# vccheng2001/DeepVCP-Pointcloud-Registration

Hardware: AMD Instinct MI355X
Metric: pairs/sec (full DeepVCP forward) at N=16384, K=64; rot/trans error vs ref (higher is better)
Workload: dtype f32

## Files before the change

### deepvcp-pointcloud-registration_amd/csrc/knn_tiled.hip

```cpp
#include "common.h"
#include "morton.h"

namespace dvcp {

constexpr int kTile = 16;
constexpr int kMaxTiles = 1024;
constexpr uint32_t kTileIdBits = 0x3FFu;
constexpr int kTiledThreads = 256;
constexpr int kBoxBatch = 1;

struct TiledLayout {
  float4* sorted;
  float4* tbox;
  float4* qsorted;
  uint32_t* qbins;
  uint32_t* qbox;
};

inline int64_t align256(int64_t x) { return (x + 255) & ~int64_t(255); }

inline TiledLayout tiled_layout(void* ws, int B, int M, int Q) {
  const int64_t T = ceil_div(M, kTile);
  char* p = static_cast<char*>(ws);
  TiledLayout L;
// ... 386 lines not shown
          const float dx = c[4 * j] - qx, dy = c[4 * j + 1] - qy, dz = c[4 * j + 2] - qz;
          d2v[j] = (dx * dx + dy * dy) + dz * dz;
          piv[j] = __float_as_uint(c[4 * j + 3]);
          const uint64_t pk = (static_cast<uint64_t>(__float_as_uint(d2v[j])) << 32) | piv[j];
          const bool cand = act & (d2v[j] < __builtin_huge_valf()) & (pk < kkey);
          todo |= __ballot(cand) != 0 ? (1u << j) : 0u;
        }
        while (todo) {
          const int j = __builtin_ctz(todo);
          todo &= todo - 1;
          const float d2 = d2v[j];
          const uint32_t pi = piv[j];
          const uint64_t pk = (static_cast<uint64_t>(__float_as_uint(d2)) << 32) | pi;
          const bool cand = act & (d2 < __builtin_huge_valf()) & (pk < kkey);
          const uint64_t m = __ballot(cand);
          if (m == 0) continue;
          ins |= m;
          const uint64_t pkc = cand ? pk : ~0ull;
          bool lt[KT];
#pragma unroll
          for (int u = 0; u < KT; ++u) lt[u] = pkc < DVCP_KK(u);
#pragma unroll
          for (int u = KT - 1; u > 0; --u) {
            kh[u] = lt[u - 1] ? kh[u - 1] : (lt[u] ? __float_as_uint(d2) : kh[u]);
            kl[u] = lt[u - 1] ? kl[u - 1] : (lt[u] ? pi : kl[u]);
          }
          kh[0] = lt[0] ? __float_as_uint(d2) : kh[0];
          kl[0] = lt[0] ? pi : kl[0];
          kkey = live ? (KT == 1 ? DVCP_KK(0) : DVCP_KK(kq)) : 0ull;
          kth = __uint_as_float(static_cast<uint32_t>(kkey >> 32));
        }
      }
      if (ins != 0) wkth = wave_max_nonneg(kth);
      }
    }
  }
  if (!live) return;
  const int64_t o = (static_cast<int64_t>(b) * Q + q) * k;
#pragma unroll
  for (int t = 0; t < KT; ++t) {
    if (t < k) {
      const bool ok = DVCP_KK(t) != kEmpty;
      const float d2 = __uint_as_float(kh[t]);
      const int i = static_cast<int>(kl[t]);
      if (dist) dist[o + t] = ok ? sqrt_rn(d2) : __builtin_huge_valf();
      if (idx) idx[o + t] = ok ? i : -1;
      if (idx64) idx64[o + t] = ok ? i : -1;
    }
  }
#undef DVCP_KK
}


#ifndef DVCP_KNN_SORD
#define DVCP_KNN_SORD 1
#endif
#ifndef DVCP_KNN_STAGE_OUT
#define DVCP_KNN_STAGE_OUT 2
#endif
constexpr int kSelBufN = 16;
constexpr int kSelSortN = 16;
constexpr int kSordWords = (kMaxTiles + 2) / 3;
#ifndef DVCP_KNN_CHUNK
#define DVCP_KNN_CHUNK 1
#endif
#ifndef DVCP_KNN_SLOAD
#define DVCP_KNN_SLOAD 1
#endif

constexpr double kKeyEmpty = __builtin_bit_cast(double, 0x3FF0000000000000ull | (0x7F800000ull << 14) | 0x3FFFull);
__device__ __forceinline__ double key_pack(float d2, uint32_t index) {
  return __builtin_bit_cast(double, 0x3FF0000000000000ull | (static_cast<uint64_t>(__float_as_uint(d2)) << 14) |
                                        static_cast<uint64_t>(index & 0x3FFFu));
}
__device__ __forceinline__ float key_d2(double kd) {
  return __uint_as_float(static_cast<uint32_t>((__builtin_bit_cast(uint64_t, kd) >> 14) & 0x7FFFFFFFull));
}
__device__ __forceinline__ int key_index(double kd) {
  return static_cast<int>(__builtin_bit_cast(uint64_t, kd) & 0x3FFFull);
}
__device__ __forceinline__ void key_ce_f64(double& a, double& b, bool asc) {
  const double lo = __builtin_fmin(a, b), hi = __builtin_fmax(a, b);
  a = asc ? lo : hi;
  b = asc ? hi : lo;
}

__device__ __forceinline__ void key_ce(uint32_t& ah, uint32_t& al, uint32_t& bh, uint32_t& bl, bool asc) {
  const uint64_t a = (static_cast<uint64_t>(ah) << 32) | al, b = (static_cast<uint64_t>(bh) << 32) | bl;
  const bool sw = asc ? (b < a) : (a < b);
  const uint32_t th = ah, tl = al;
  ah = sw ? bh : ah;
  al = sw ? bl : al;
  bh = sw ? th : bh;
  bl = sw ? tl : bl;
}

template <int R>
__global__ __launch_bounds__(kTiledThreads) __attribute__((amdgpu_waves_per_eu(3))) void knn_sel_query_kernel(const float4* __restrict__ sorted,
                                                                      const float4* __restrict__ tbox,
                                                                      const float4* __restrict__ qsorted, int M,
                                                                      int Q, int k,
                                                                      float* __restrict__ dist,
                                                                      int32_t* __restrict__ idx,
                                                                      int64_t* __restrict__ idx64, int B8) {
  constexpr int KT = 32;
  const int lane = threadIdx.x & 63, wave = threadIdx.x >> 6;
  int b = blockIdx.y, bx = blockIdx.x;
  if ((B8 & 1) != 0) {
    const int lin = static_cast<int>(blockIdx.y * gridDim.x + blockIdx.x);
    const int xo = lin & 7, slot = lin >> 3;
    b = xo + 8 * (slot / static_cast<int>(gridDim.x));
    bx = slot % static_cast<int>(gridDim.x);
  }
  const int T = (M + kTile - 1) / kTile;
  __shared__ uint3 hbox[kMaxTiles];
  __shared__ uint32_t sord[kTiledThreads / kWave][kSordWords];
  __shared__ double sbuf[kTiledThreads / kWave][kSelBufN][kWave];
  __shared__ float4 stile[kTiledThreads / kWave][kTile];
  {
    const float4* tbg = tbox + static_cast<int64_t>(b) * T * 2;
    for (int i = threadIdx.x; i < T; i += kTiledThreads) hbox[i] = pack_hbox(tbg[2 * i], tbg[2 * i + 1]);
    __syncthreads();
  }
  const int sq0 = __builtin_amdgcn_readfirstlane((bx * (kTiledThreads / kWave) + wave) * kWave);
  const int sq = sq0 + lane;
  if (sq0 >= Q) return;
  const bool live = sq < Q;
  const float4 qrow = live ? qsorted[static_cast<int64_t>(b) * Q + sq] : make_float4(0.f, 0.f, 0.f, 0.f);
  const float qx = qrow.x, qy = qrow.y, qz = qrow.z;
  auto out_row = [&]() {
    const int sqn = sq0 + knn_fresh_lane();
    return __float_as_int(qsorted[static_cast<int64_t>(b) * Q + sqn].w);
  };
  float wl[3] = {live ? qx : __builtin_huge_valf(), live ? qy : __builtin_huge_valf(),
                 live ? qz : __builtin_huge_valf()};
  float wh[3] = {live ? qx : -__builtin_huge_valf(), live ? qy : -__builtin_huge_valf(),
                 live ? qz : -__builtin_huge_valf()};
#pragma unroll
  for (int a = 0; a < 3; ++a) {
    wl[a] = __int_as_float(__builtin_amdgcn_readfirstlane(__float_as_int(-wave_max_nonneg_signed(-wl[a]))));
    wh[a] = __int_as_float(__builtin_amdgcn_readfirstlane(__float_as_int(wave_max_nonneg_signed(wh[a]))));
  }
  uint32_t keys[R];
#pragma unroll
  for (int r = 0; r < R; ++r) {
    const int t = r * 64 + lane;
    if (t < T) {
      const float lb = hbox_lb2(hbox[t], wl[0], wl[1], wl[2], wh[0], wh[1], wh[2]);
      keys[r] = (__float_as_uint(lb) & ~kTileIdBits) | static_cast<uint32_t>(t);
    } else {
      keys[r] = 0xFFFFFFFFu;
    }
  }
  wave_bitonic<R>(keys);

  double tk[KT];
#pragma unroll
  for (int t = 0; t < KT; ++t) tk[t] = kKeyEmpty;
  float kth = live ? __builtin_huge_valf() : 0.0f;
  float wkth = wave_max_nonneg(kth);
  int fill = 0;
  double(*mybuf)[kWave] = sbuf[wave];
#ifdef DVCP_KNN_DIAG
  uint64_t dg_t0 = __builtin_readcyclecounter(), dg_merge_clk = 0, dg_skip_clk = 0, dg_prev = 0;
  int dg_kind = -1;
  int dg_scanned = 0, dg_active = 0, dg_merges = 0, dg_appends = 0;
#endif

  auto merge = [&]() {
    const int n = static_cast<int>(wave_umax_i(static_cast<uint32_t>(fill)));
    if (n == 0) return;
#ifdef DVCP_KNN_DIAG
    const uint64_t dg_m0 = __builtin_readcyclecounter();
    ++dg_merges;
#endif
    double bk[kSelSortN];
#pragma unroll
    for (int i = 0; i < kSelSortN; ++i) {
      bk[i] = kKeyEmpty;
      if (i < kSelBufN && i < n) {
        const double e = mybuf[i][lane];
        bk[i] = i < fill ? e : bk[i];
      }
    }
#pragma unroll
    for (int kk = 2; kk <= kSelSortN; kk <<= 1)
#pragma unroll
      for (int j = kk >> 1; j > 0; j >>= 1)
#pragma unroll
        for (int i = 0; i < kSelSortN; ++i) {
          const int l = i ^ j;
          if (l > i) key_ce_f64(bk[i], bk[l], (i & kk) == 0);
        }
#pragma unroll
    for (int i = KT - kSelSortN; i < KT; ++i) tk[i] = __builtin_fmin(tk[i], bk[KT - 1 - i]);
#pragma unroll
    for (int j = KT >> 1; j > 0; j >>= 1)
#pragma unroll
      for (int i = 0; i < KT; ++i) {
        const int l = i ^ j;
        if (l > i) key_ce_f64(tk[i], tk[l], true);
      }
    kth = live ? key_d2(tk[KT - 1]) : 0.0f;
    wkth = wave_max_nonneg(kth);
    fill = 0;
#ifdef DVCP_KNN_DIAG
    dg_merge_clk += __builtin_readcyclecounter() - dg_m0;
// ... 29 lines not shown
#pragma unroll
    for (int j = 0; j < kTile; ++j) {
      c[3 * j] = bc(4 * j);
      c[3 * j + 1] = bc(4 * j + 1);
      c[3 * j + 2] = bc(4 * j + 2);
    }
#endif
    auto d2_of = [&](int j) {
      const float dx = c[3 * j] - qx, dy = c[3 * j + 1] - qy, dz = c[3 * j + 2] - qz;
      return (dx * dx + dy * dy) + dz * dz;
    };
    uint32_t cm = 0;
    const float kf = fminf(kth, __builtin_bit_cast(float, 0x7F7FFFFFu));
#pragma unroll
    for (int j = 0; j < kTile; ++j) cm |= (act && d2_of(j) <= kf) ? (1u << j) : 0u;
    if (wave_umax_i(static_cast<uint32_t>(fill + __popc(cm))) > static_cast<uint32_t>(kSelBufN)) {
      merge();
      const float kf2 = fminf(kth, __builtin_bit_cast(float, 0x7F7FFFFFu));
#pragma unroll
      for (int j = 0; j < kTile; ++j) cm &= d2_of(j) <= kf2 ? ~0u : ~(1u << j);
    }
    if (__ballot(cm != 0) != 0) {
#if DVCP_KNN_SLOAD
      reinterpret_cast<float*>(stile[wave])[lane] = P[static_cast<int64_t>(t) * (4 * kTile) + lane];
#else
      reinterpret_cast<float*>(stile[wave])[lane] = v_cur;
#endif
      __builtin_amdgcn_wave_barrier();
      uint32_t my = cm;
      while (__ballot(my != 0) != 0) {
        if (my != 0) {
          const int j = __builtin_ctz(my);
          my &= my - 1;
#ifdef DVCP_KNN_DIAG
          ++dg_appends;
#endif
          const float4 pt = stile[wave][j];
          const float dx = pt.x - qx, dy = pt.y - qy, dz = pt.z - qz;
          mybuf[fill][lane] = key_pack((dx * dx + dy * dy) + dz * dz, __float_as_uint(pt.w));
          ++fill;
        }
      }
      __builtin_amdgcn_wave_barrier();
    }
  };
  auto visit = [&](uint32_t key) {
    const int t = static_cast<int>(key & kTileIdBits);
    const float lbq = hbox_lb2(hbox[t], qx, qy, qz, qx, qy, qz);
    float v = 0.0f;
    if (__ballot(live & (lbq <= kth)) != 0) v = P[static_cast<int64_t>(t) * (4 * kTile) + lane];
    visit_loaded(key, lbq, v);
  };

#if DVCP_KNN_CHUNK
  constexpr int kKnnSub = 4, kSubLanes = kWave / kKnnSub;
  float gl[3] = {wl[0], wl[1], wl[2]}, gh[3] = {wh[0], wh[1], wh[2]};
  {
    float a[3] = {live ? qx : __builtin_huge_valf(), live ? qy : __builtin_huge_valf(),
                  live ? qz : __builtin_huge_valf()};
    float z[3] = {live ? qx : -__builtin_huge_valf(), live ? qy : -__builtin_huge_valf(),
                  live ? qz : -__builtin_huge_valf()};
#pragma unroll
    for (int ax = 0; ax < 3; ++ax)
#pragma unroll
      for (int off = kSubLanes / 2; off > 0; off >>= 1) {
        a[ax] = fminf(a[ax], __shfl_xor(a[ax], off, kWave));
        z[ax] = fmaxf(z[ax], __shfl_xor(z[ax], off, kWave));
      }
#pragma unroll
    for (int ax = 0; ax < 3; ++ax) {
      gl[ax] = a[ax];
      gh[ax] = z[ax];
    }
  }
  __shared__ float4 sgbox[kTiledThreads / kWave][kKnnSub][2];
  if ((lane & (kSubLanes - 1)) == 0) {
    sgbox[wave][lane / kSubLanes][0] = make_float4(gl[0], gl[1], gl[2], 0.0f);
    sgbox[wave][lane / kSubLanes][1] = make_float4(gh[0], gh[1], gh[2], 0.0f);
  }
#if DVCP_KNN_SORD
  for (int i = lane; i < kSordWords; i += kWave) sord[wave][i] = 0u;
  __builtin_amdgcn_wave_barrier();
#pragma unroll
  for (int r = 0; r < R; ++r) {
    const int p = r * 64 + lane;
    if (p < T) atomicOr(&sord[wave][p / 3], (keys[r] & kTileIdBits) << (10 * (p % 3)));
  }
  __builtin_amdgcn_wave_barrier();
#endif
  bool stop = false;
#pragma unroll 1
  for (int base = 0; base < T && !stop; base += kWave) {
    const bool inr = base + lane < T;
#if DVCP_KNN_SORD
    const int pos = base + lane;
    const int tt = inr ? static_cast<int>((sord[wave][pos / 3] >> (10 * (pos % 3))) & kTileIdBits) : 0;
    const uint3 hb = hbox[tt];
    const uint32_t mykey = inr ? (__float_as_uint(hbox_lb2(hb, wl[0], wl[1], wl[2], wh[0], wh[1], wh[2])) &
                                  ~kTileIdBits) | static_cast<uint32_t>(tt)
                               : 0xFFFFFFFFu;
#else
    const uint32_t mykey = keys[base >> 6];
    const int tt = inr ? static_cast<int>(mykey & kTileIdBits) : 0;
    const uint3 hb = hbox[tt < T ? tt : 0];
#endif
    const float klb = __uint_as_float(mykey & ~kTileIdBits);
    const uint64_t over = __ballot(!inr || klb > wkth);
    const int lim = over ? __builtin_ctzll(over) : kWave;
    float gk = kth;
#pragma unroll
    for (int off = kSubLanes / 2; off > 0; off >>= 1) gk = fmaxf(gk, __shfl_xor(gk, off, kWave));
    float gks[kKnnSub];
#pragma unroll
    for (int g = 0; g < kKnnSub; ++g) gks[g] = __int_as_float(__builtin_amdgcn_readlane(__float_as_int(gk), g * kSubLanes));
    const float blx = half_lo(hb.x), bly = half_hi(hb.x), blz = half_lo(hb.y);
    const float bhx = half_hi(hb.y), bhy = half_lo(hb.z), bhz = half_hi(hb.z);
    bool pass = false;
#pragma unroll
    for (int g = 0; g < kKnnSub; ++g) {
      const float4 lo = sgbox[wave][g][0], hi = sgbox[wave][g][1];
      pass |= box_box_lb2(lo.x, lo.y, lo.z, hi.x, hi.y, hi.z, blx, bly, blz, bhx, bhy, bhz) <= gks[g];
    }
    uint64_t cand = __ballot(pass && inr) & (lim >= kWave ? ~0ull : ((1ull << lim) - 1ull));
    if (lim < kWave) stop = true;
    while (cand) {
      const int i = __builtin_ctzll(cand);
      cand &= cand - 1ull;
      const uint32_t key = static_cast<uint32_t>(__builtin_amdgcn_readlane(static_cast<int>(mykey), i));
      if (__uint_as_float(key & ~kTileIdBits) > wkth) {
        stop = true;
        break;
      }
      visit(key);
    }
  }
#else
  uint32_t key_next = T > 0 ? static_cast<uint32_t>(__builtin_amdgcn_readlane(static_cast<int>(keys[0]), 0)) : 0u;
#pragma unroll 1
  for (int pos = 0; pos < T; ++pos) {
#ifdef DVCP_KNN_DIAG
    {
      const uint64_t now = __builtin_readcyclecounter();
      if (dg_kind == 0) dg_skip_clk += now - dg_prev;
      dg_prev = now;
      dg_kind = 0;
    }
#endif
    const uint32_t key = key_next;
    if (pos + 1 < T)
      key_next = static_cast<uint32_t>(__builtin_amdgcn_readlane(static_cast<int>(keys[(pos + 1) >> 6]), (pos + 1) & 63));
    if (__uint_as_float(key & ~kTileIdBits) > wkth) break;
    visit(key);
  }
#endif
  merge();
#ifdef DVCP_KNN_DIAG
  const uint64_t dg_total = __builtin_readcyclecounter() - dg_t0;
  uint32_t app_sum = static_cast<uint32_t>(dg_appends);
  for (int off = 32; off > 0; off >>= 1) app_sum += __shfl_xor(app_sum, off, kWave);
#endif
#ifndef DVCP_KNN_DIAG
  if constexpr (DVCP_KNN_STAGE_OUT == 2) {
    if (dist && idx && !idx64 && k == KT) {
      if (!live) return;
      const int qo = out_row();
      float4* dr = reinterpret_cast<float4*>(dist + (static_cast<int64_t>(b) * Q + qo) * 32);
      int4* ir = reinterpret_cast<int4*>(idx + (static_cast<int64_t>(b) * Q + qo) * 32);
#pragma unroll
      for (int v = 0; v < KT / 4; ++v) {
        float dv[4];
        int iv[4];
#pragma unroll
        for (int e = 0; e < 4; ++e) {
          const double kv = tk[4 * v + e];
          const bool ok = kv != kKeyEmpty;
          dv[e] = ok ? sqrt_rn(key_d2(kv)) : __builtin_huge_valf();
          iv[e] = ok ? key_index(kv) : -1;
        }
        dr[v] = make_float4(dv[0], dv[1], dv[2], dv[3]);
        ir[v] = make_int4(iv[0], iv[1], iv[2], iv[3]);
      }
      return;
    }
  }
  if constexpr (DVCP_KNN_STAGE_OUT == 1) {
    if (dist && idx && !idx64 && k == KT) {
      const int qo = live ? out_row() : -1;
      float* stage = reinterpret_cast<float*>(sbuf[wave]);
#pragma unroll
      for (int part = 0; part < 2; ++part) {
#pragma unroll
        for (int half = 0; half < 2; ++half) {
          if ((lane >> 5) == half) {
#pragma unroll
            for (int t = 0; t < KT; ++t) {
              const bool ok = tk[t] != kKeyEmpty;
              const float v = part == 0 ? (ok ? sqrt_rn(key_d2(tk[t])) : __builtin_huge_valf())
                                        : __int_as_float(ok ? key_index(tk[t]) : -1);
              stage[(lane & 31) * 33 + t] = v;
            }
          }
          __builtin_amdgcn_wave_barrier();
          __builtin_amdgcn_fence(__ATOMIC_ACQ_REL, "wavefront");
#pragma unroll
          for (int it = 0; it < 4; ++it) {
            const int row = it * 8 + (lane >> 3), piece = lane & 7;
            const int rq = __shfl(qo, half * 32 + row, kWave);
            const float* sr = stage + row * 33 + 4 * piece;
            const float4 v = make_float4(sr[0], sr[1], sr[2], sr[3]);
            if (rq >= 0) {
              float* dst = part == 0 ? dist : reinterpret_cast<float*>(idx);
              reinterpret_cast<float4*>(dst + (static_cast<int64_t>(b) * Q + rq) * 32)[piece] = v;
            }
          }
          __builtin_amdgcn_wave_barrier();
          __builtin_amdgcn_fence(__ATOMIC_ACQ_REL, "wavefront");
        }
      }
      return;
    }
  }
#endif
  if (!live) return;
  const int qo = out_row();
  const int64_t o = (static_cast<int64_t>(b) * Q + qo) * k;
#ifdef DVCP_KNN_DIAG
  if (lane == 0 && dist && k == 32) {
    dist[o + 0] = static_cast<float>(dg_scanned);
    dist[o + 1] = static_cast<float>(dg_active);
    dist[o + 2] = static_cast<float>(dg_merges);
    dist[o + 3] = static_cast<float>(app_sum);
    dist[o + 4] = static_cast<float>(dg_total);
    dist[o + 5] = static_cast<float>(dg_merge_clk);
    dist[o + 6] = static_cast<float>(dg_skip_clk);
    dist[o + 31] = -12345.0f;
    return;
  }
#endif
#pragma unroll
  for (int t = 0; t < KT; ++t) {
    if (t < k) {
      const bool ok = tk[t] != kKeyEmpty;
      const float d2 = key_d2(tk[t]);
      const int i = key_index(tk[t]);
      if (dist) dist[o + t] = ok ? sqrt_rn(d2) : __builtin_huge_valf();
      if (idx) idx[o + t] = ok ? i : -1;
      if (idx64) idx64[o + t] = ok ? i : -1;
    }
  }
}

}

extern "C" int64_t dvcp_knn_tiled_workspace_bytes(int B, int M, int Q) {
  if (B < 0 || M < 0 || Q < 0) return -1;
  const int64_t T = dvcp::ceil_div(M, dvcp::kTile);
  return dvcp::align256(16 * int64_t(B) * T * dvcp::kTile) + dvcp::align256(32 * int64_t(B) * T) +
         dvcp::align256(16 * int64_t(B) * Q) + dvcp::align256(dvcp::tiled_zeroed_bytes(B));
}

static int knn_tiled_impl(int dtype, const void* ref, int64_t rb, int64_t rc, int64_t rn, int M, const void* qry,
                          int64_t qb, int64_t qc, int64_t qn, int Q, int B, int k, void* workspace, float* dist,
                          int32_t* idx, int64_t* idx64, void* stream, bool insertion) {
  DVCP_REQUIRE(ref && qry && workspace, "dvcp_knn_tiled: null pointer");
  DVCP_REQUIRE(k > 0 && k <= 32 && M >= 0 && Q >= 0 && B >= 0 && B <= 65535, "dvcp_knn_tiled: bad sizes");
  DVCP_REQUIRE(M <= dvcp::kMaxTiles * dvcp::kTile, "dvcp_knn_tiled: M=%d > %d", M, dvcp::kMaxTiles * dvcp::kTile);
  DVCP_REQUIRE(dtype == DVCP_F32 || dtype == DVCP_F64, "dvcp_knn_tiled: bad dtype %d", dtype);
  if (B == 0 || Q == 0) return DVCP_OK;
  hipStream_t st = static_cast<hipStream_t>(stream);
  const dvcp::TiledLayout L = dvcp::tiled_layout(workspace, B, M, Q);
  if (hipMemsetAsync(L.qbins, 0, dvcp::tiled_zeroed_bytes(B), st) != hipSuccess) {
    dvcp::set_error("dvcp_knn_tiled: memset failed");
    return DVCP_EHIP;
  }
  const dim3 qgrid(dvcp::ceil_div(Q, dvcp::kQSortItems), B), bgrid(1 + qgrid.x, B);
  if (dtype == DVCP_F32) {
    const dvcp::PointsView<float> qv{static_cast<const float*>(qry), qb, qc, qn};
    hipLaunchKernelGGL((dvcp::knn_qbox_kernel<float>), qgrid, dim3(dvcp::kBuildThreads), 0, st, qv, Q, L.qbox);
    hipLaunchKernelGGL((dvcp::knn_qhist_kernel<float>), qgrid, dim3(dvcp::kBuildThreads), 0, st, qv, Q, L.qbox,
                       L.qbins);
    hipLaunchKernelGGL(dvcp::knn_qscan_kernel, dim3(B), dim3(dvcp::kBuildThreads), 0, st, L.qbins);
    hipLaunchKernelGGL((dvcp::knn_tiled_build_kernel<float>), bgrid, dim3(dvcp::kBuildThreads), 0, st,
                       dvcp::PointsView<float>{static_cast<const float*>(ref), rb, rc, rn}, M, qv, Q, L);
  } else {
    const dvcp::PointsView<double> qv{static_cast<const double*>(qry), qb, qc, qn};
    hipLaunchKernelGGL((dvcp::knn_qbox_kernel<double>), qgrid, dim3(dvcp::kBuildThreads), 0, st, qv, Q, L.qbox);
    hipLaunchKernelGGL((dvcp::knn_qhist_kernel<double>), qgrid, dim3(dvcp::kBuildThreads), 0, st, qv, Q, L.qbox,
                       L.qbins);
    hipLaunchKernelGGL(dvcp::knn_qscan_kernel, dim3(B), dim3(dvcp::kBuildThreads), 0, st, L.qbins);
    hipLaunchKernelGGL((dvcp::knn_tiled_build_kernel<double>), bgrid, dim3(dvcp::kBuildThreads), 0, st,
                       dvcp::PointsView<double>{static_cast<const double*>(ref), rb, rc, rn}, M, qv, Q, L);
  }
  if (int e = dvcp::launch_status("dvcp_knn_tiled(build)")) return e;
  const int T = dvcp::ceil_div(M, dvcp::kTile);
  dim3 grid(dvcp::ceil_div(Q, dvcp::kTiledThreads), B);
  const int xcd = B % 8 == 0 ? 1 : 0;
#define DVCP_KNNS(RR)                                                                                             \
  if (k > 16 && T <= 64 * RR) {                                                                                   \
    hipLaunchKernelGGL((dvcp::knn_sel_query_kernel<RR>), grid, dim3(dvcp::kTiledThreads), 0, st, L.sorted,         \
                       L.tbox, L.qsorted, M, Q, k, dist, idx, idx64, xcd);                                         \
    return dvcp::launch_status("dvcp_knn_tiled(select)");                                                         \
  }
  if (!insertion) {
    DVCP_KNNS(1)
    DVCP_KNNS(2)
    DVCP_KNNS(4)
    DVCP_KNNS(8)
    DVCP_KNNS(16)
  }
#undef DVCP_KNNS
#define DVCP_KNNT(KK, RR)                                                                                          \
  if (k <= KK && T <= 64 * RR) {                                                                                   \
    hipLaunchKernelGGL((dvcp::knn_tiled_query_kernel<KK, RR>), grid, dim3(dvcp::kTiledThreads), 0, st, L.sorted,   \
                       L.tbox, L.qsorted, M, Q, k, dist, idx, idx64, xcd);                                          \
    return dvcp::launch_status("dvcp_knn_tiled(query)");                                                           \
  }
  DVCP_KNNT(1, 1)
  DVCP_KNNT(1, 16)
  DVCP_KNNT(8, 1)
  DVCP_KNNT(8, 16)
  DVCP_KNNT(16, 16)
  DVCP_KNNT(32, 1)
  DVCP_KNNT(32, 2)
  DVCP_KNNT(32, 4)
  DVCP_KNNT(32, 8)
  DVCP_KNNT(32, 16)
#undef DVCP_KNNT
  dvcp::set_error("dvcp_knn_tiled: unsupported k=%d", k);
  return DVCP_EINVAL;
}

extern "C" int dvcp_knn_tiled(int dtype, const void* ref, int64_t rb, int64_t rc, int64_t rn, int M, const void* qry,
                              int64_t qb, int64_t qc, int64_t qn, int Q, int B, int k, void* workspace, float* dist,
                              int32_t* idx, int64_t* idx64, void* stream) {
  return knn_tiled_impl(dtype, ref, rb, rc, rn, M, qry, qb, qc, qn, Q, B, k, workspace, dist, idx, idx64, stream, false);
}

extern "C" int dvcp_knn_tiled_insert(int dtype, const void* ref, int64_t rb, int64_t rc, int64_t rn, int M,
                                     const void* qry, int64_t qb, int64_t qc, int64_t qn, int Q, int B, int k,
                                     void* workspace, float* dist, int32_t* idx, int64_t* idx64, void* stream) {
  return knn_tiled_impl(dtype, ref, rb, rc, rn, M, qry, qb, qc, qn, Q, B, k, workspace, dist, idx, idx64, stream, true);
}
```

### deepvcp-pointcloud-registration_amd/dvcp/_lib.py

```python
import contextlib
import ctypes
import os

import torch

_HERE = os.path.dirname(os.path.abspath(__file__))
LIB_PATH = os.environ.get("DVCP_LIB_PATH") or os.path.join(_HERE, "libdvcp_hip.so")

F32, F64 = 0, 1
ABI_VERSION = 4
_P = ctypes.c_void_p
_I = ctypes.c_int
_L = ctypes.c_int64
_D = ctypes.c_double

SIGNATURES = {
    "dvcp_fps": [_I, _P, _L, _L, _L, _I, _I, _I, _P, _P, _P, _P],
    "dvcp_fps_ws": [_I, _P, _L, _L, _L, _I, _I, _I, _P, _P, _P, _P, _P, _P],
    "dvcp_fps_parts": [_I, _P, _L, _L, _L, _I, _I, _I, _P, _P, _P, _P, _L, _P, _I, _P],
    "dvcp_fps_step_floor": [_I, _I, _P, _P],
    "dvcp_fps_pair": [_I, _P, _L, _L, _L, _I, _I, _P, _P, _P, _P, _P, _P, _P, _P],
    "dvcp_fps_split_probe": [_I, _P, _L, _L, _L, _I, _I, _I, _P, _P, _P, _P, _P, ctypes.c_uint32, _I, _P],
    "dvcp_ball_query": [_I, _P, _L, _L, _L, _I, _P, _L, _L, _L, _I, _I, _D, _I, _P, _P, _P, _P],
    "dvcp_ball_query_ws": [_I, _P, _L, _L, _L, _I, _P, _L, _L, _L, _I, _I, _D, _I, _P, _P, _P, _P, _P],
    "dvcp_square_distance": [_I, _P, _L, _L, _L, _I, _P, _L, _L, _L, _I, _I, _P, _P],
    "dvcp_sa_group_mlp": [_I, _P, _L, _L, _L, _I, _P, _L, _L, _L, _I, _I, _I, _P, _L, _L, _L, _I,
                          _P, _P, _I, _I, _P, _P, _P, _P],
    "dvcp_sa_group_mlp_ws": [_I, _P, _L, _L, _L, _I, _P, _L, _L, _L, _I, _I, _I, _P, _L, _L, _L, _I,
                             _P, _P, _I, _I, _P, _P, _P, _P, _P],
    "dvcp_sa_group_mlp_rows_ws": [_I, _P, _L, _L, _L, _I, _P, _L, _L, _L, _I, _I, _P, _L, _L, _I, _I, _P,
                                  _P, _P, _I, _I, _P, _P, _P, _P, _P],
    "dvcp_fe_head": [_P, _I, _P, _P, _P, _P],
    "dvcp_fe_head_rows": [_P, _P, _I, _I, _I, _P, _P, _P, _P],
    "dvcp_weighting": [_P, _I, _P, _P, _P],
    "dvcp_topk": [_P, _I, _I, _I, _P, _P],
    "dvcp_src_keypoints": [_I, _P, _P, _I, _P, _I, _I, _P, _D, _I, _P, _L, _P, _P, _P, _P],
    "dvcp_voxelize": [_I, _P, _L, _L, _L, _I, _I, _D, _D, _I, _P, _P, _P],
    "dvcp_knn": [_I, _P, _L, _L, _L, _I, _P, _L, _L, _L, _I, _I, _I, _P, _P, _P, _P],
    "dvcp_knn_grid": [_I, _P, _L, _L, _L, _I, _P, _L, _L, _L, _I, _I, _I, _P, _P, _P, _P, _P],
    "dvcp_knn_tiled": [_I, _P, _L, _L, _L, _I, _P, _L, _L, _L, _I, _I, _I, _P, _P, _P, _P, _P],
    "dvcp_knn_tiled_insert": [_I, _P, _L, _L, _L, _I, _P, _L, _L, _L, _I, _I, _I, _P, _P, _P, _P, _P],
    "dvcp_dfe": [_I, _P, _L, _P, _P, _P],
    "dvcp_dfe_tgt": [_I, _P, _L, _L, _L, _I, _P, _P, _P, _P, _I, _I, _P, _P, _P],
    "dvcp_points_pack4": [_P, _L, _L, _L, _I, _I, _P, _P],
    "dvcp_dfe_tgt_f16": [_I, _P, _L, _L, _L, _I, _P, _P, _P, _P, _I, _I, _P, _P, _P],
    "dvcp_dfe_tgt_literal": [_I, _P, _L, _L, _L, _I, _P, _P, _P, _P, _I, _I, _P, _P, _P],
    "dvcp_cpg": [_P, _P, _L, _L, _L, _P, _I, _I, _P, _P, _P, _P],
    "dvcp_rigid_transform": [_P, _P, _I, _I, _P, _P, _P],
    "dvcp_paper_pose": [_P, _P, _P, _I, _I, _I, _D, _P, _P, _P, _P, _P, _P],
    "dvcp_paper_pose_backward": [_P, _P, _P, _I, _I, _I, _D, _P, _P, _D, _P, _P, _P, _P],
    "dvcp_feature_propagation": [_P, _L, _L, _L, _I, _P, _L, _L, _L, _I, _I, _P, _L, _L, _L, _I, _P, _L, _L, _I,
                                 _I, _P, _P, _P, _P, _P],
    "dvcp_group_rows": [_P, _L, _L, _L, _I, _P, _L, _L, _L, _P, _L, _L, _I, _P, _P, _I, _I, _D, _I, _P, _P],
    "dvcp_cpg1d": [_P, _P, _P, _I, _I, _P, _P, _P, _P],
    "dvcp_svd_optimization": [_P, _P, _P, _P, _I, _I, _P, _P, _P, _P, _P, _P],
    "dvcp_deepvcp_loss": [_P, _P, _P, _P, _I, _I, _D, _P, _P, _P, _P, _P],
    "dvcp_registration_error": [_P, _P, _P, _L, _P, _L, _I, _P, _P, _P],
    "dvcp_rigid_apply": [_I, _P, _L, _L, _L, _I, _I, _I, _P, _P, _L, _P, _P],
    "dvcp_svd_optimization_backward": [_P, _P, _P, _P, _I, _I, _P, _P, _D, _P, _P],
    "dvcp_dfe_backward": [_I, _P, _L, _P, _P, _P, _P, _P, _P],
    "dvcp_dfe_tgt_backward": [_I, _P, _L, _L, _L, _I, _P, _P, _P, _P, _I, _I, _P, _P, _P, _P, _P, _P],
    "dvcp_src_keypoints_backward": [_I, _P, _I, _P, _I, _I, _P, _D, _I, _P, _P, _P],
    "dvcp_cpg_backward": [_P, _P, _L, _L, _L, _P, _I, _I, _P, _P, _P, _P, _P, _P, _P],
    "dvcp_sa_group_mlp_backward": [_I, _P, _L, _L, _L, _I, _P, _L, _L, _L, _I, _I, _I, _P, _L, _L, _L, _I,
                                   _P, _P, _I, _I, _P, _P, _P, _P, _P, _P, _P, _P],
    "dvcp_fe_head_backward": [_P, _I, _P, _P, _P, _P, _P, _P],
    "dvcp_sa_bn_stats": [_I, _P, _L, _L, _L, _I, _P, _L, _L, _L, _I, _I, _I, _P, _L, _L, _L, _I,
                         _P, _P, _I, _I, _P, _P, _I, _P, _P, _P, _P],
    "dvcp_sa_bn_backward": [_I, _P, _L, _L, _L, _I, _P, _L, _L, _L, _I, _I, _I, _P, _L, _L, _L, _I,
                            _P, _P, _I, _I, _P, _P, _P, _I, _P, _P, _P, _P, _P, _P],
    "dvcp_sa_bn_zrows": [_I, _P, _L, _L, _L, _I, _P, _L, _L, _L, _I, _I, _I, _P, _L, _L, _L, _I,
                         _P, _P, _I, _I, _P, _P, _P, _P],
    "dvcp_sa_bnm_pre": [_P, _L, _L, _I, _I, _I, _P, _P, _P, _P],
    "dvcp_sa_bnm_pass": [_I, _P, _L, _L, _L, _I, _P, _L, _L, _L, _I, _I, _P, _L, _L, _L, _I, _P, _P, _I, _I, _P,
                         _P, _P, _P, _P, _P, _P, _P, _P, _P, _P, _P],
}

_lib = None


def load():
    global _lib
    if _lib is not None:
        return _lib
    if not os.path.exists(LIB_PATH):
        raise RuntimeError(
            f"dvcp: HIP library not built ({LIB_PATH} missing). Run `make -j16` in "
            "deepvcp-pointcloud-registration_amd/ or __graft_entry__.build().")
    lib = ctypes.CDLL(LIB_PATH, mode=ctypes.RTLD_GLOBAL)
    lib.dvcp_last_error.restype = ctypes.c_char_p
    lib.dvcp_last_error.argtypes = []
    lib.dvcp_abi_version.restype = ctypes.c_int
    lib.dvcp_abi_version.argtypes = []
    if lib.dvcp_abi_version() != ABI_VERSION:
# ... 187 lines not shown
```

### include/dvcp.h

```cpp
#ifndef DVCP_H
#define DVCP_H
#include <stdint.h>

#ifdef __cplusplus
extern "C" {
#endif

#define DVCP_F32 0
#define DVCP_F64 1

#define DVCP_OK 0
#define DVCP_EINVAL (-1)
#define DVCP_EHIP (-2)

#define DVCP_ABI_VERSION 4

const char* dvcp_last_error(void);
int dvcp_abi_version(void);

int dvcp_fps(int dtype, const void* xyz, int64_t sb, int64_t sc, int64_t sn, int B, int N,
             int npoint, const int64_t* start, int64_t* out_idx, void* out_xyz, void* stream);

int dvcp_fps_ws(int dtype, const void* xyz, int64_t sb, int64_t sc, int64_t sn, int B, int N,
                int npoint, const int64_t* start, int64_t* out_idx, void* out_xyz, float* ws,
// ... 36 lines not shown
                      const int32_t* count, const int32_t* list, int nsample,
                      int nlayer, const int* chans, const float* params, float* out,
                      void* stream);

int64_t dvcp_sa_group_mlp_workspace_bytes(int B, int N, int S, int nlayer, const int* chans);
int dvcp_sa_group_mlp_ws(int dtype, const void* xyz, int64_t sb, int64_t sc, int64_t sn, int N,
                         const void* ctr, int64_t cb, int64_t cc, int64_t cn, int S, int B,
                         int feat_dtype, const void* feat, int64_t fb, int64_t fd, int64_t fn, int D,
                         const int32_t* count, const int32_t* list, int nsample,
                         int nlayer, const int* chans, const float* params, float* out,
                         void* workspace, void* stream);

int dvcp_sa_group_mlp_rows_ws(int dtype, const void* xyz, int64_t sb, int64_t sc, int64_t sn, int N,
                              const void* ctr, int64_t cb, int64_t cc, int64_t cn, int S, int B,
                              const float* feat, int64_t fb, int64_t fn, int Nf, int D,
                              const int64_t* feat_rows, const int32_t* count, const int32_t* list,
                              int nsample, int nlayer, const int* chans, const float* params, float* out,
                              void* workspace, void* stream);

int dvcp_fe_head(const float* x, int P, const float* params, float* feat, float* score,
                 void* stream);

int dvcp_fe_head_rows(const float* x, const int64_t* rows, int S, int Nx, int P, const float* params,
                      float* feat, float* score, void* stream);

int dvcp_weighting(const float* feat, int P, const float* params, float* score, void* stream);

int dvcp_topk(const float* score, int B, int S, int K, int64_t* idx, void* stream);

int dvcp_src_keypoints(int dtype, const void* fe_xyz, const float* fe_feat, int S,
                       const int64_t* topk, int B, int K, const int64_t* kstart,
                       double radius, int nsample, const double* R_init, int64_t r_b,
                       void* keypts, float* src_cat, double* moved, void* stream);

int dvcp_voxelize(int dtype, const void* pts, int64_t pb, int64_t pc, int64_t pn, int B, int Kp,
                  double r, double s, int G, float* cand, int32_t* err, void* stream);

int dvcp_knn(int dtype, const void* ref, int64_t rb, int64_t rc, int64_t rn, int M,
             const void* qry, int64_t qb, int64_t qc, int64_t qn, int Q, int B, int k,
             float* dist, int32_t* idx, int64_t* idx64, void* stream);

int dvcp_knn_grid(int dtype, const void* ref, int64_t rb, int64_t rc, int64_t rn, int M,
                  const void* qry, int64_t qb, int64_t qc, int64_t qn, int Q, int B, int k,
                  void* workspace, float* dist, int32_t* idx, int64_t* idx64, void* stream);
int64_t dvcp_knn_grid_workspace_bytes(int B, int M);

int dvcp_knn_tiled(int dtype, const void* ref, int64_t rb, int64_t rc, int64_t rn, int M,
                   const void* qry, int64_t qb, int64_t qc, int64_t qn, int Q, int B, int k,
                   void* workspace, float* dist, int32_t* idx, int64_t* idx64, void* stream);
int dvcp_knn_tiled_insert(int dtype, const void* ref, int64_t rb, int64_t rc, int64_t rn, int M,
                          const void* qry, int64_t qb, int64_t qc, int64_t qn, int Q, int B, int k,
                          void* workspace, float* dist, int32_t* idx, int64_t* idx64, void* stream);
int64_t dvcp_knn_tiled_workspace_bytes(int B, int M, int Q);

int dvcp_dfe(int x_dtype, const void* X, int64_t R, const float* params, float* out,
             void* stream);

int dvcp_dfe_tgt(int dtype, const void* ref_xyz, int64_t rb, int64_t rc, int64_t rn, int M,
                 const float* ref_feat, const float* cand, const float* dist, const int32_t* idx,
                 int B, int Q, const float* params, float* out, void* stream);

int dvcp_points_pack4(const float* xyz, int64_t sb, int64_t sc, int64_t sn, int M, int B, float* out,
                      void* stream);

int dvcp_dfe_tgt_f16(int dtype, const void* ref_xyz, int64_t rb, int64_t rc, int64_t rn, int M,
                     const uint16_t* ref_feat, const float* cand, const float* dist, const int32_t* idx,
                     int B, int Q, const float* params, float* out, void* stream);

int dvcp_dfe_tgt_literal(int dtype, const void* ref_xyz, int64_t rb, int64_t rc, int64_t rn, int M,
                         const float* ref_feat, const float* cand, const float* dist,
                         const int32_t* idx, int B, int Q, const float* params, float* out,
                         void* stream);

int64_t dvcp_sa_group_mlp_backward_workspace_bytes(int B, int S, int nlayer, const int* chans);
int dvcp_sa_group_mlp_backward(int dtype, const void* xyz, int64_t sb, int64_t sc, int64_t sn, int N,
                               const void* ctr, int64_t cb, int64_t cc, int64_t cn, int S, int B,
                               int feat_dtype, const void* feat, int64_t fb, int64_t fd, int64_t fn,
                               int D, const int32_t* count, const int32_t* list, int nsample,
                               int nlayer, const int* chans, const float* params,
                               const float* bnstat, const float* grad_out, float* grad_feat,
                               void* workspace, float* grad_params, void* stream);

int64_t dvcp_sa_bn_pack_floats(int nlayer, const int* chans);
int64_t dvcp_sa_bn_workspace_bytes(int B, int S, int nlayer, const int* chans);
int64_t dvcp_sa_bn_rows_floats(int B, int S, int nsample, int nlayer, const int* chans);
int64_t dvcp_sa_bn_feat_workspace_bytes(int B, int S, int nsample, int N, int D);
int64_t dvcp_sa_bn_zrows_floats(int B, int S, int nsample, int nlayer, const int* chans);
int dvcp_sa_bn_zrows(int dtype, const void* xyz, int64_t sb, int64_t sc, int64_t sn, int N,
                     const void* ctr, int64_t cb, int64_t cc, int64_t cn, int S, int B,
                     int feat_dtype, const void* feat, int64_t fb, int64_t fd, int64_t fn, int D,
                     const int32_t* count, const int32_t* list, int nsample, int nlayer,
                     const int* chans, const float* pack, float* zrows, void* stream);
int dvcp_sa_bn_stats(int dtype, const void* xyz, int64_t sb, int64_t sc, int64_t sn, int N,
                     const void* ctr, int64_t cb, int64_t cc, int64_t cn, int S, int B,
                     int feat_dtype, const void* feat, int64_t fb, int64_t fd, int64_t fn, int D,
                     const int32_t* count, const int32_t* list, int nsample, int nlayer,
                     const int* chans, const float* pack, int layer, void* workspace,
                     double* sums, float* zrows, void* stream);
int dvcp_sa_bn_backward(int dtype, const void* xyz, int64_t sb, int64_t sc, int64_t sn, int N,
                        const void* ctr, int64_t cb, int64_t cc, int64_t cn, int S, int B,
                        int feat_dtype, const void* feat, int64_t fb, int64_t fd, int64_t fn,
                        int D, const int32_t* count, const int32_t* list, int nsample, int nlayer,
                        const int* chans, const float* pack, const float* zrows, int mode,
                        const float* grad_out, float* grad_feat, void* workspace, double* sums,
                        float* rows, void* stream);

// ... 91 lines not shown
```

Baseline: 2588.

## Replace per-wave bitonic tile sort with bucketed counting order and upper-bound pruning

The full wave bitonic sort of tile lower-bound keys is replaced by a 256-bucket counting sort keyed on float exponent bits. Tiles whose lower bound exceeds the second-smallest upper bound are pruned up front, so only the kept tiles are scanned, and termination is decided per bucket. The sub-group max reduction now uses DPP row ops instead of xor shuffles. A probe kernel and C entry point are added to dump the ordering. Because ordering within a bucket is only approximate, the early-stop logic had to change to skip per tile rather than break, and it adds LDS atomics.

```diff
diff --git a/deepvcp-pointcloud-registration_amd/csrc/knn_tiled.hip b/deepvcp-pointcloud-registration_amd/csrc/knn_tiled.hip
--- a/deepvcp-pointcloud-registration_amd/csrc/knn_tiled.hip
+++ b/deepvcp-pointcloud-registration_amd/csrc/knn_tiled.hip
@@ -462,18 +462,12 @@
 }
 
 
-#ifndef DVCP_KNN_SORD
-#define DVCP_KNN_SORD 1
-#endif
 #ifndef DVCP_KNN_STAGE_OUT
 #define DVCP_KNN_STAGE_OUT 2
 #endif
 constexpr int kSelBufN = 16;
 constexpr int kSelSortN = 16;
 constexpr int kSordWords = (kMaxTiles + 2) / 3;
-#ifndef DVCP_KNN_CHUNK
-#define DVCP_KNN_CHUNK 1
-#endif
 #ifndef DVCP_KNN_SLOAD
 #define DVCP_KNN_SLOAD 1
 #endif
@@ -503,6 +497,137 @@
   al = sw ? bl : al;
   bh = sw ? th : bh;
   bl = sw ? tl : bl;
+}
+
+constexpr int kOrdBuckets = 256;
+constexpr int kOrdShift = 19;
+constexpr float kUbMargin = 1.0f + 0x1p-20f;
+
+__device__ __forceinline__ int knn_bucket_top(float range) {
+  return static_cast<int>(__float_as_uint(range) >> kOrdShift);
+}
+__device__ __forceinline__ int knn_bucket(float lb, int top) {
+  const int below = top - static_cast<int>(__float_as_uint(lb) >> kOrdShift);
+  return max(0, kOrdBuckets - 1 - max(0, below));
+}
+
+__device__ __forceinline__ float knn_tile_lb(const uint3& h, const float (&wl)[3], const float (&wh)[3]) {
+  return __uint_as_float(__float_as_uint(hbox_lb2(h, wl[0], wl[1], wl[2], wh[0], wh[1], wh[2])) & ~kTileIdBits);
+}
+
+__device__ __forceinline__ float hbox_ub2(const uint3& h, float alx, float aly, float alz, float ahx, float ahy,
+                                          float ahz) {
+  const float blx = half_lo(h.x), bly = half_hi(h.x), blz = half_lo(h.y);
+  const float bhx = half_hi(h.y), bhy = half_lo(h.z), bhz = half_hi(h.z);
+  const float fx = fmaxf(bhx - alx, ahx - blx), fy = fmaxf(bhy - aly, ahy - bly), fz = fmaxf(bhz - alz, ahz - blz);
+  const float u = ((fx * fx + fy * fy) + fz * fz) * kUbMargin;
+  const float s = ((fabsf(blx) + fabsf(bly)) + fabsf(blz)) + ((fabsf(bhx) + fabsf(bhy)) + fabsf(bhz));
+  return s < __builtin_huge_valf() ? u : __builtin_huge_valf();
+}
+
+__device__ __forceinline__ float wave_min_nonneg(float x) {
+  return __uint_as_float(~wave_umax_i(~__float_as_uint(x)));
+}
+
+__device__ __forceinline__ bool knn_wave_box(bool live, float qx, float qy, float qz, float (&wl)[3], float (&wh)[3]) {
+  const float q[3] = {qx, qy, qz};
+#pragma unroll
+  for (int a = 0; a < 3; ++a) {
+    const float lo = live ? q[a] : __builtin_huge_valf(), hi = live ? q[a] : -__builtin_huge_valf();
+    wl[a] = __int_as_float(__builtin_amdgcn_readfirstlane(__float_as_int(-wave_max_nonneg_signed(-lo))));
+    wh[a] = __int_as_float(__builtin_amdgcn_readfirstlane(__float_as_int(wave_max_nonneg_signed(hi))));
+  }
+  return __ballot(live && !((fabsf(qx) + fabsf(qy)) + fabsf(qz) < __builtin_huge_valf())) == 0;
+}
+
+struct WaveOrder {
+  float b0;
+  int top;
+  int kept;
+};
+
+template <int R>
+__device__ __forceinline__ WaveOrder knn_wave_order(const uint3* hbox, int T, int M, const float (&wl)[3],
+                                                    const float (&wh)[3], bool qfinite, uint32_t* cnt,
+                                                    uint32_t* sordw, float (&lbv)[R]) {
+  const int lane = threadIdx.x & 63;
+  const float inf = __builtin_huge_valf();
+  for (int i = lane; i < kSordWords; i += kWave) sordw[i] = 0u;
+  constexpr int kPer = kOrdBuckets / kWave;
+#pragma unroll
+  for (int j = 0; j < kPer; ++j) cnt[j * kWave + lane] = 0u;
+  float m1 = inf, m2 = inf, lbmax = 0.0f;
+#pragma unroll
+  for (int r = 0; r < R; ++r) {
+    lbv[r] = 0.0f;
+    if (r * 64 < T) {
+      const int t = r * 64 + lane;
+      if (t < T) {
+        const uint3 hb = hbox[t];
+        lbv[r] = knn_tile_lb(hb, wl, wh);
+        lbmax = fmaxf(lbmax, lbv[r] < inf ? lbv[r] : 0.0f);
+        const float ub = (t + 1) * kTile <= M ? hbox_ub2(hb, wl[0], wl[1], wl[2], wh[0], wh[1], wh[2]) : inf;
+        const float u = ub >= 0.0f ? ub : inf;
+        m2 = fminf(m2, fmaxf(m1, u));
+        m1 = fminf(m1, u);
+      }
+    }
+  }
+  WaveOrder o;
+  {
+    const float g1 = wave_min_nonneg(m1);
+    const uint64_t own = __ballot(m1 == g1);
+    const int owner = own ? __builtin_ctzll(own) : 0;
+    const float g2 = wave_min_nonneg(lane == owner ? m2 : m1);
+    o.b0 = __int_as_float(__builtin_amdgcn_readfirstlane(__float_as_int(qfinite ? g2 : inf)));
+  }
+  o.top = __builtin_amdgcn_readfirstlane(knn_bucket_top(o.b0 < inf ? o.b0 : wave_max_nonneg(lbmax)));
+  __builtin_amdgcn_fence(__ATOMIC_RELEASE, "wavefront");
+  __builtin_amdgcn_wave_barrier();
+#pragma unroll
+  for (int r = 0; r < R; ++r)
+    if (r * 64 < T) {
+      const int t = r * 64 + lane;
+      if (t < T && !(lbv[r] > o.b0)) atomicAdd(&cnt[knn_bucket(lbv[r], o.top)], 1u);
+    }
+  __builtin_amdgcn_fence(__ATOMIC_ACQ_REL, "wavefront");
+  __builtin_amdgcn_wave_barrier();
+  {
+    uint32_t c[kPer], sum = 0u;
+#pragma unroll
+    for (int j = 0; j < kPer; ++j) {
+      c[j] = cnt[lane * kPer + j];
+      sum += c[j];
+    }
+    uint32_t incl = sum;
+#pragma unroll
+    for (int off = 1; off < kWave; off <<= 1) {
+      const uint32_t up = static_cast<uint32_t>(__shfl_up(static_cast<int>(incl), off, kWave));
+      incl += lane >= off ? up : 0u;
+    }
+    o.kept = __builtin_amdgcn_readlane(static_cast<int>(incl), 63);
+    __builtin_amdgcn_wave_barrier();
+    uint32_t base = incl - sum;
+#pragma unroll
+    for (int j = 0; j < kPer; ++j) {
+      cnt[lane * kPer + j] = base;
+      base += c[j];
+    }
+  }
+  __builtin_amdgcn_fence(__ATOMIC_ACQ_REL, "wavefront");
+  __builtin_amdgcn_wave_barrier();
+#pragma unroll
+  for (int r = 0; r < R; ++r)
+    if (r * 64 < T) {
+      const int t = r * 64 + lane;
+      if (t < T && !(lbv[r] > o.b0)) {
+        const uint32_t p = atomicAdd(&cnt[knn_bucket(lbv[r], o.top)], 1u);
+        atomicOr(&sordw[p / 3], static_cast<uint32_t>(t) << (10 * (p % 3)));
+      }
+    }
+  __builtin_amdgcn_fence(__ATOMIC_ACQ_REL, "wavefront");
+  __builtin_amdgcn_wave_barrier();
+  return o;
 }
 
 template <int R>
@@ -542,27 +667,13 @@
     const int sqn = sq0 + knn_fresh_lane();
     return __float_as_int(qsorted[static_cast<int64_t>(b) * Q + sqn].w);
   };
-  float wl[3] = {live ? qx : __builtin_huge_valf(), live ? qy : __builtin_huge_valf(),
-                 live ? qz : __builtin_huge_valf()};
-  float wh[3] = {live ? qx : -__builtin_huge_valf(), live ? qy : -__builtin_huge_valf(),
-                 live ? qz : -__builtin_huge_valf()};
-#pragma unroll
-  for (int a = 0; a < 3; ++a) {
-    wl[a] = __int_as_float(__builtin_amdgcn_readfirstlane(__float_as_int(-wave_max_nonneg_signed(-wl[a]))));
-    wh[a] = __int_as_float(__builtin_amdgcn_readfirstlane(__float_as_int(wave_max_nonneg_signed(wh[a]))));
-  }
-  uint32_t keys[R];
-#pragma unroll
-  for (int r = 0; r < R; ++r) {
-    const int t = r * 64 + lane;
-    if (t < T) {
-      const float lb = hbox_lb2(hbox[t], wl[0], wl[1], wl[2], wh[0], wh[1], wh[2]);
-      keys[r] = (__float_as_uint(lb) & ~kTileIdBits) | static_cast<uint32_t>(t);
-    } else {
-      keys[r] = 0xFFFFFFFFu;
-    }
-  }
-  wave_bitonic<R>(keys);
+  float wl[3], wh[3];
+  const bool qfinite = knn_wave_box(live, qx, qy, qz, wl, wh);
+  WaveOrder ord;
+  {
+    float lbv[R];
+    ord = knn_wave_order<R>(hbox, T, M, wl, wh, qfinite, reinterpret_cast<uint32_t*>(sbuf[wave]), sord[wave], lbv);
+  }
 
   double tk[KT];
 #pragma unroll
@@ -698,7 +809,6 @@
     visit_loaded(key, lbq, v);
   };
 
-#if DVCP_KNN_CHUNK
   constexpr int kKnnSub = 4, kSubLanes = kWave / kKnnSub;
   float gl[3] = {wl[0], wl[1], wl[2]}, gh[3] = {wh[0], wh[1], wh[2]};
   {
@@ -724,41 +834,27 @@
     sgbox[wave][lane / kSubLanes][0] = make_float4(gl[0], gl[1], gl[2], 0.0f);
     sgbox[wave][lane / kSubLanes][1] = make_float4(gh[0], gh[1], gh[2], 0.0f);
   }
-#if DVCP_KNN_SORD
-  for (int i = lane; i < kSordWords; i += kWave) sord[wave][i] = 0u;
-  __builtin_amdgcn_wave_barrier();
-#pragma unroll
-  for (int r = 0; r < R; ++r) {
-    const int p = r * 64 + lane;
-    if (p < T) atomicOr(&sord[wave][p / 3], (keys[r] & kTileIdBits) << (10 * (p % 3)));
-  }
-  __builtin_amdgcn_wave_barrier();
-#endif
   bool stop = false;
 #pragma unroll 1
-  for (int base = 0; base < T && !stop; base += kWave) {
-    const bool inr = base + lane < T;
-#if DVCP_KNN_SORD
+  for (int base = 0; base < ord.kept && !stop; base += kWave) {
+    const bool inr = base + lane < ord.kept;
     const int pos = base + lane;
     const int tt = inr ? static_cast<int>((sord[wave][pos / 3] >> (10 * (pos % 3))) & kTileIdBits) : 0;
     const uint3 hb = hbox[tt];
-    const uint32_t mykey = inr ? (__float_as_uint(hbox_lb2(hb, wl[0], wl[1], wl[2], wh[0], wh[1], wh[2])) &
-                                  ~kTileIdBits) | static_cast<uint32_t>(tt)
-                               : 0xFFFFFFFFu;
-#else
-    const uint32_t mykey = keys[base >> 6];
-    const int tt = inr ? static_cast<int>(mykey & kTileIdBits) : 0;
-    const uint3 hb = hbox[tt < T ? tt : 0];
-#endif
-    const float klb = __uint_as_float(mykey & ~kTileIdBits);
-    const uint64_t over = __ballot(!inr || klb > wkth);
-    const int lim = over ? __builtin_ctzll(over) : kWave;
-    float gk = kth;
-#pragma unroll
-    for (int off = kSubLanes / 2; off > 0; off >>= 1) gk = fmaxf(gk, __shfl_xor(gk, off, kWave));
+    const float mylb = knn_tile_lb(hb, wl, wh);
+    const uint32_t mykey = __float_as_uint(mylb) | static_cast<uint32_t>(tt);
+    const int blast = __builtin_amdgcn_readlane(knn_bucket(mylb, ord.top), min(kWave, ord.kept - base) - 1);
+    static_assert(kSubLanes == 16, "one DPP row per lane group");
+    uint32_t gk = __float_as_uint(kth);
+    gk = dpp_max_u<0x111, 0xF>(gk);
+    gk = dpp_max_u<0x112, 0xF>(gk);
+    gk = dpp_max_u<0x114, 0xF>(gk);
+    gk = dpp_max_u<0x118, 0xF>(gk);
     float gks[kKnnSub];
 #pragma unroll
-    for (int g = 0; g < kKnnSub; ++g) gks[g] = __int_as_float(__builtin_amdgcn_readlane(__float_as_int(gk), g * kSubLanes));
+    for (int g = 0; g < kKnnSub; ++g)
+      gks[g] = __uint_as_float(static_cast<uint32_t>(
+          __builtin_amdgcn_readlane(static_cast<int>(gk), g * kSubLanes + kSubLanes - 1)));
     const float blx = half_lo(hb.x), bly = half_hi(hb.x), blz = half_lo(hb.y);
     const float bhx = half_hi(hb.y), bhy = half_lo(hb.z), bhz = half_hi(hb.z);
     bool pass = false;
@@ -767,38 +863,16 @@
       const float4 lo = sgbox[wave][g][0], hi = sgbox[wave][g][1];
       pass |= box_box_lb2(lo.x, lo.y, lo.z, hi.x, hi.y, hi.z, blx, bly, blz, bhx, bhy, bhz) <= gks[g];
     }
-    uint64_t cand = __ballot(pass && inr) & (lim >= kWave ? ~0ull : ((1ull << lim) - 1ull));
-    if (lim < kWave) stop = true;
+    uint64_t cand = __ballot(pass && inr && !(mylb > wkth));
     while (cand) {
       const int i = __builtin_ctzll(cand);
       cand &= cand - 1ull;
       const uint32_t key = static_cast<uint32_t>(__builtin_amdgcn_readlane(static_cast<int>(mykey), i));
-      if (__uint_as_float(key & ~kTileIdBits) > wkth) {
-        stop = true;
-        break;
-      }
+      if (__uint_as_float(key & ~kTileIdBits) > wkth) continue;
       visit(key);
     }
-  }
-#else
-  uint32_t key_next = T > 0 ? static_cast<uint32_t>(__builtin_amdgcn_readlane(static_cast<int>(keys[0]), 0)) : 0u;
-#pragma unroll 1
-  for (int pos = 0; pos < T; ++pos) {
-#ifdef DVCP_KNN_DIAG
-    {
-      const uint64_t now = __builtin_readcyclecounter();
-      if (dg_kind == 0) dg_skip_clk += now - dg_prev;
-      dg_prev = now;
-      dg_kind = 0;
-    }
-#endif
-    const uint32_t key = key_next;
-    if (pos + 1 < T)
-      key_next = static_cast<uint32_t>(__builtin_amdgcn_readlane(static_cast<int>(keys[(pos + 1) >> 6]), (pos + 1) & 63));
-    if (__uint_as_float(key & ~kTileIdBits) > wkth) break;
-    visit(key);
-  }
-#endif
+    stop = blast > knn_bucket(wkth, ord.top);
+  }
   merge();
 #ifdef DVCP_KNN_DIAG
   const uint64_t dg_total = __builtin_readcyclecounter() - dg_t0;
@@ -896,6 +970,58 @@
   }
 }
 
+template <int R>
+__global__ __launch_bounds__(kTiledThreads) void knn_order_probe_kernel(const float4* __restrict__ tbox,
+                                                                        const float4* __restrict__ qsorted, int M,
+                                                                        int Q, int32_t* __restrict__ info,
+                                                                        int32_t* __restrict__ order,
+                                                                        float* __restrict__ lbs,
+                                                                        int32_t* __restrict__ buckets, int B8) {
+  const int lane = threadIdx.x & 63, wave = threadIdx.x >> 6;
+  int b = blockIdx.y, bx = blockIdx.x;
+  if ((B8 & 1) != 0) {
+    const int lin = static_cast<int>(blockIdx.y * gridDim.x + blockIdx.x);
+    const int xo = lin & 7, slot = lin >> 3;
+    b = xo + 8 * (slot / static_cast<int>(gridDim.x));
+    bx = slot % static_cast<int>(gridDim.x);
+  }
+  const int T = (M + kTile - 1) / kTile;
+  __shared__ uint3 hbox[kMaxTiles];
+  __shared__ uint32_t sord[kTiledThreads / kWave][kSordWords];
+  __shared__ uint32_t scnt[kTiledThreads / kWave][kOrdBuckets];
+  {
+    const float4* tbg = tbox + static_cast<int64_t>(b) * T * 2;
+    for (int i = threadIdx.x; i < T; i += kTiledThreads) hbox[i] = pack_hbox(tbg[2 * i], tbg[2 * i + 1]);
+    __syncthreads();
+  }
+  const int sq0 = __builtin_amdgcn_readfirstlane((bx * (kTiledThreads / kWave) + wave) * kWave);
+  const int sq = sq0 + lane;
+  if (sq0 >= Q) return;
+  const bool live = sq < Q;
+  const float4 qrow = live ? qsorted[static_cast<int64_t>(b) * Q + sq] : make_float4(0.f, 0.f, 0.f, 0.f);
+  float wl[3], wh[3];
+  const bool qfinite = knn_wave_box(live, qrow.x, qrow.y, qrow.z, wl, wh);
+  float lbv[R];
+  const WaveOrder ord = knn_wave_order<R>(hbox, T, M, wl, wh, qfinite, scnt[wave], sord[wave], lbv);
+  const int64_t row = static_cast<int64_t>(b) * ((Q + kWave - 1) / kWave) + sq0 / kWave;
+  if (lane == 0) {
+    info[row * 4 + 0] = T - ord.kept;
+    info[row * 4 + 1] = ord.kept;
+    info[row * 4 + 2] = ord.b0 < __builtin_huge_valf() ? 1 : 0;
+    info[row * 4 + 3] = __float_as_int(ord.b0);
+  }
+  for (int p = lane; p < T; p += kWave)
+    order[row * T + p] = p < ord.kept ? static_cast<int>((sord[wave][p / 3] >> (10 * (p % 3))) & kTileIdBits) : -1;
+#pragma unroll
+  for (int r = 0; r < R; ++r) {
+    const int t = r * 64 + lane;
+    if (t < T) {
+      lbs[row * T + t] = lbv[r];
+      buckets[row * T + t] = lbv[r] > ord.b0 ? -1 : knn_bucket(lbv[r], ord.top);
+    }
+  }
+}
+
 }
 
 extern "C" int64_t dvcp_knn_tiled_workspace_bytes(int B, int M, int Q) {
@@ -905,16 +1031,9 @@
          dvcp::align256(16 * int64_t(B) * Q) + dvcp::align256(dvcp::tiled_zeroed_bytes(B));
 }
 
-static int knn_tiled_impl(int dtype, const void* ref, int64_t rb, int64_t rc, int64_t rn, int M, const void* qry,
-                          int64_t qb, int64_t qc, int64_t qn, int Q, int B, int k, void* workspace, float* dist,
-                          int32_t* idx, int64_t* idx64, void* stream, bool insertion) {
-  DVCP_REQUIRE(ref && qry && workspace, "dvcp_knn_tiled: null pointer");
-  DVCP_REQUIRE(k > 0 && k <= 32 && M >= 0 && Q >= 0 && B >= 0 && B <= 65535, "dvcp_knn_tiled: bad sizes");
-  DVCP_REQUIRE(M <= dvcp::kMaxTiles * dvcp::kTile, "dvcp_knn_tiled: M=%d > %d", M, dvcp::kMaxTiles * dvcp::kTile);
-  DVCP_REQUIRE(dtype == DVCP_F32 || dtype == DVCP_F64, "dvcp_knn_tiled: bad dtype %d", dtype);
-  if (B == 0 || Q == 0) return DVCP_OK;
-  hipStream_t st = static_cast<hipStream_t>(stream);
-  const dvcp::TiledLayout L = dvcp::tiled_layout(workspace, B, M, Q);
+static int knn_tiled_build(int dtype, const void* ref, int64_t rb, int64_t rc, int64_t rn, int M, const void* qry,
+                           int64_t qb, int64_t qc, int64_t qn, int Q, int B, const dvcp::TiledLayout& L,
+                           hipStream_t st) {
   if (hipMemsetAsync(L.qbins, 0, dvcp::tiled_zeroed_bytes(B), st) != hipSuccess) {
     dvcp::set_error("dvcp_knn_tiled: memset failed");
     return DVCP_EHIP;
@@ -937,7 +1056,20 @@
     hipLaunchKernelGGL((dvcp::knn_tiled_build_kernel<double>), bgrid, dim3(dvcp::kBuildThreads), 0, st,
                        dvcp::PointsView<double>{static_cast<const double*>(ref), rb, rc, rn}, M, qv, Q, L);
   }
-  if (int e = dvcp::launch_status("dvcp_knn_tiled(build)")) return e;
+  return dvcp::launch_status("dvcp_knn_tiled(build)");
+}
+
+static int knn_tiled_impl(int dtype, const void* ref, int64_t rb, int64_t rc, int64_t rn, int M, const void* qry,
+                          int64_t qb, int64_t qc, int64_t qn, int Q, int B, int k, void* workspace, float* dist,
+                          int32_t* idx, int64_t* idx64, void* stream, bool insertion) {
+  DVCP_REQUIRE(ref && qry && workspace, "dvcp_knn_tiled: null pointer");
+  DVCP_REQUIRE(k > 0 && k <= 32 && M >= 0 && Q >= 0 && B >= 0 && B <= 65535, "dvcp_knn_tiled: bad sizes");
+  DVCP_REQUIRE(M <= dvcp::kMaxTiles * dvcp::kTile, "dvcp_knn_tiled: M=%d > %d", M, dvcp::kMaxTiles * dvcp::kTile);
+  DVCP_REQUIRE(dtype == DVCP_F32 || dtype == DVCP_F64, "dvcp_knn_tiled: bad dtype %d", dtype);
+  if (B == 0 || Q == 0) return DVCP_OK;
+  hipStream_t st = static_cast<hipStream_t>(stream);
+  const dvcp::TiledLayout L = dvcp::tiled_layout(workspace, B, M, Q);
+  if (int e = knn_tiled_build(dtype, ref, rb, rc, rn, M, qry, qb, qc, qn, Q, B, L, st)) return e;
   const int T = dvcp::ceil_div(M, dvcp::kTile);
   dim3 grid(dvcp::ceil_div(Q, dvcp::kTiledThreads), B);
   const int xcd = B % 8 == 0 ? 1 : 0;
@@ -987,3 +1119,34 @@
                                      void* workspace, float* dist, int32_t* idx, int64_t* idx64, void* stream) {
   return knn_tiled_impl(dtype, ref, rb, rc, rn, M, qry, qb, qc, qn, Q, B, k, workspace, dist, idx, idx64, stream, true);
 }
+
+extern "C" int dvcp_knn_tiled_order_probe(int dtype, const void* ref, int64_t rb, int64_t rc, int64_t rn, int M,
+                                          const void* qry, int64_t qb, int64_t qc, int64_t qn, int Q, int B,
+                                          void* workspace, int32_t* info, int32_t* order, float* lb,
+                                          int32_t* bucket, void* stream) {
+  DVCP_REQUIRE(ref && qry && workspace && info && order && lb && bucket, "dvcp_knn_tiled_order_probe: null pointer");
+  DVCP_REQUIRE(M > 0 && Q > 0 && B > 0 && B <= 65535, "dvcp_knn_tiled_order_probe: bad sizes");
+  DVCP_REQUIRE(M <= dvcp::kMaxTiles * dvcp::kTile, "dvcp_knn_tiled_order_probe: M=%d > %d", M,
+               dvcp::kMaxTiles * dvcp::kTile);
+  DVCP_REQUIRE(dtype == DVCP_F32 || dtype == DVCP_F64, "dvcp_knn_tiled_order_probe: bad dtype %d", dtype);
+  hipStream_t st = static_cast<hipStream_t>(stream);
+  const dvcp::TiledLayout L = dvcp::tiled_layout(workspace, B, M, Q);
+  if (int e = knn_tiled_build(dtype, ref, rb, rc, rn, M, qry, qb, qc, qn, Q, B, L, st)) return e;
+  const int T = dvcp::ceil_div(M, dvcp::kTile);
+  const dim3 grid(dvcp::ceil_div(Q, dvcp::kTiledThreads), B);
+  const int xcd = B % 8 == 0 ? 1 : 0;
+#define DVCP_KNNP(RR)                                                                                            \
+  if (T <= 64 * RR) {                                                                                            \
+    hipLaunchKernelGGL((dvcp::knn_order_probe_kernel<RR>), grid, dim3(dvcp::kTiledThreads), 0, st, L.tbox,        \
+                       L.qsorted, M, Q, info, order, lb, bucket, xcd);                                            \
+    return dvcp::launch_status("dvcp_knn_tiled_order_probe");                                                    \
+  }
+  DVCP_KNNP(1)
+  DVCP_KNNP(2)
+  DVCP_KNNP(4)
+  DVCP_KNNP(8)
+  DVCP_KNNP(16)
+#undef DVCP_KNNP
+  dvcp::set_error("dvcp_knn_tiled_order_probe: unsupported M=%d", M);
+  return DVCP_EINVAL;
+}
diff --git a/deepvcp-pointcloud-registration_amd/dvcp/_lib.py b/deepvcp-pointcloud-registration_amd/dvcp/_lib.py
--- a/deepvcp-pointcloud-registration_amd/dvcp/_lib.py
+++ b/deepvcp-pointcloud-registration_amd/dvcp/_lib.py
@@ -40,6 +40,7 @@
     "dvcp_knn_grid": [_I, _P, _L, _L, _L, _I, _P, _L, _L, _L, _I, _I, _I, _P, _P, _P, _P, _P],
     "dvcp_knn_tiled": [_I, _P, _L, _L, _L, _I, _P, _L, _L, _L, _I, _I, _I, _P, _P, _P, _P, _P],
     "dvcp_knn_tiled_insert": [_I, _P, _L, _L, _L, _I, _P, _L, _L, _L, _I, _I, _I, _P, _P, _P, _P, _P],
+    "dvcp_knn_tiled_order_probe": [_I, _P, _L, _L, _L, _I, _P, _L, _L, _L, _I, _I, _P, _P, _P, _P, _P, _P],
     "dvcp_dfe": [_I, _P, _L, _P, _P, _P],
     "dvcp_dfe_tgt": [_I, _P, _L, _L, _L, _I, _P, _P, _P, _P, _I, _I, _P, _P, _P],
     "dvcp_points_pack4": [_P, _L, _L, _L, _I, _I, _P, _P],
diff --git a/include/dvcp.h b/include/dvcp.h
--- a/include/dvcp.h
+++ b/include/dvcp.h
@@ -112,6 +112,10 @@
                           const void* qry, int64_t qb, int64_t qc, int64_t qn, int Q, int B, int k,
                           void* workspace, float* dist, int32_t* idx, int64_t* idx64, void* stream);
 int64_t dvcp_knn_tiled_workspace_bytes(int B, int M, int Q);
+int dvcp_knn_tiled_order_probe(int dtype, const void* ref, int64_t rb, int64_t rc, int64_t rn, int M,
+                               const void* qry, int64_t qb, int64_t qc, int64_t qn, int Q, int B,
+                               void* workspace, int32_t* info, int32_t* order, float* lb,
+                               int32_t* bucket, void* stream);
 
 int dvcp_dfe(int x_dtype, const void* X, int64_t R, const float* params, float* out,
              void* stream);
```

New measurement: 2638 (median of 6 runs). +2.0%, better.
